# kcleal/fslr

Hardware: AMD Instinct MI355X
Metric: Jaccard pair-compares/sec + HBM GB/s vs roofline, 1M-read interval cluster (higher is better)
Workload: dtype int32

## Files before the change

### fslr_amd/csrc/capi.hip

```cpp
#include <algorithm>
#include <atomic>
#include <cstdint>
#include <cstdlib>
#include <cstring>
#include <string>
#include <thread>
#include <vector>

#include "fslr_hip.h"
#include "ctx.hpp"
#include "kernels.hpp"

using namespace fslr;

namespace {

int alloc_errw(fslr_ctx* c, int cap);

int ensure_capacity(fslr_ctx* c, int64_t n, int64_t ni, int n_chroms) {
  int rc;
  if (n > c->cap_n) {
    if ((rc = dalloc(c, &c->rmeta, n)) || (rc = dalloc(c, &c->rlen8, n)) || (rc = dalloc(c, &c->fwd, n)) ||
        (rc = dalloc(c, &c->parent, n)) || (rc = dalloc(c, &c->forest, n)) ||
        (rc = dalloc(c, &c->heavy, n)) ||
// ... 740 lines not shown
  b.rmeta = c->rmeta;
  b.iv = c->iv;
  b.shard = c->shard;
  b.n_shards = c->n_shards;
  b.dchrom = c->filter_active ? c->fdchrom : c->have_data_pos ? c->dchrom : nullptr;
  b.drec = c->filter_active ? c->fdrec : c->have_data_pos ? c->drec : nullptr;
  b.dgate = c->filter_active ? c->fdgate : c->dgate;
  b.data_pos = c->data_pos;
  b.chist = c->chist;
  b.keys = c->keys;
  b.keys2 = c->keys2;
  b.vals = c->vals;
  b.vals2 = c->vals2;
  b.s_start = c->s_start;
  b.endkey = c->endkey;
  b.pmaxkey = c->pmaxkey;
  b.temp = c->temp;
  b.temp_bytes = c->temp_bytes;
  b.crange = c->filter_active ? c->crange_f : c->crange;
  b.qpos = c->qpos;
  b.rng_s = c->rng_s;
  b.swin = c->swin;
  b.tile_tests = nullptr;
  b.idx4 = c->idx4;
  b.idx_gate = c->idx_gate;
  return b;
}

__global__ void k_peek(const unsigned long long* counters, const int* err, long long* out) {
  if (threadIdx.x == 0) {
    out[0] = static_cast<long long>(counters[kEdgeCount]);
    out[1] = err[0];
    out[2] = err[3];
    out[3] = err[kErrZdCount];
  }
}

int fslr::peek_counts(fslr_ctx* c, long long out[4]) {
  if (!c->sw_total) {
    HIP_TRY(c, hipHostMalloc(reinterpret_cast<void**>(&c->sw_total), 16 * sizeof(long long), hipHostMallocMapped));
    HIP_TRY(c, hipHostGetDevicePointer(reinterpret_cast<void**>(&c->sw_total_dev), c->sw_total, 0));
  }
  k_peek<<<1, 64, 0, c->stream>>>(c->counters, c->errw, c->sw_total_dev + 4);
  HIP_TRY(c, hipGetLastError());
  HIP_TRY(c, hipStreamSynchronize(c->stream));
  const volatile long long* v = c->sw_total + 4;
// ... 34 lines not shown
int fslr::ensure_walk_index(fslr_ctx* c) {
  if (!c->index_built || c->index_full) return FSLR_OK;
  if (c->filter_active) return fail(c, FSLR_ERR_STATE, "the walk engine needs every chromosome's index");
  if (int rc = ensure_keys(c, false)) return rc;
  HIP_TRY(c, launch_index_walk_parts(index_bufs(c), static_cast<int>(c->n), static_cast<int>(c->ni), c->stream));
  c->index_full = true;
  return FSLR_OK;
}

extern "C" {

int fslr_build_index(fslr_ctx* c) {
  if (!c) return FSLR_ERR_INVALID;
  if (!c->reads_set) return fail(c, FSLR_ERR_STATE, "fslr_set_reads first");
  HIP_TRY(c, hipSetDevice(c->device));
  if (c->prof_phases) HIP_TRY(c, hipEventRecord(c->ev[0], c->stream));
  const bool full = !c->filter_active && !(c->have_data_pos && c->n_chroms <= 64 && c->n_shards == 1);
  const int nch = c->filter_active ? c->n_chroms_f : c->n_chroms;
  IndexBufs ib = index_bufs(c);
  const bool tt = !full && ib.dchrom && nch <= 64 && c->n_shards == 1;
  c->idx_tt_valid = false;
  if (tt) {
    const int64_t tiles = (c->ni_idx + 63) / 64 + 1;
    if (tiles > c->idx_tt_cap) {
      if (int rc = dalloc(c, &c->idx_tt, tiles)) return rc;
      c->idx_tt_cap = tiles;
    }
    ib.tile_tests = c->idx_tt;
  }
  HIP_TRY(c, launch_build_index(ib, static_cast<int>(c->n), static_cast<int>(c->ni_idx), nch, full, c->stream));
  c->idx_tt_valid = tt;
  c->index_lean = !full && index_bufs(c).dchrom && nch <= 64;
  c->lean_keys = false;
  c->lean_starts = false;
  c->built_n_chroms = nch;
  if (c->prof_phases) HIP_TRY(c, hipEventRecord(c->ev[1], c->stream));
  c->t_index_rec = c->prof_phases;
  c->index_built = true;
  ++c->index_gen;
  c->index_full = full;
  c->bwd_ranges = full;
  c->built_shard = c->shard;
  c->built_n_shards = c->n_shards;
  return FSLR_OK;
}

static int query_impl(fslr_ctx* c, const fslr_params* p, int64_t a_begin, int64_t a_end, int shard, int n_shards);

int fslr_query(fslr_ctx* c, const fslr_params* p, int64_t a_begin, int64_t a_end) {
  if (!c || !p || !p->pass_table) return FSLR_ERR_INVALID;
  if (a_begin < 0 || a_end > c->n || a_begin > a_end) return fail(c, FSLR_ERR_INVALID, "bad read range");
// ... 46 lines not shown
  if ((rc = ensure_grp(c))) return rc;
  s.grp = c->grp;
  s.rmeta = c->rmeta;
  s.rlen8 = c->rlen8;
  s.idx4 = c->idx4;
  s.idx_gate = c->idx_gate;
  s.rng_s = c->rng_s;
  s.swin = c->swin;
  s.umax = c->umax;
  s.ni = static_cast<int>(nix);
  if (c->filter_active && c->pf_on && c->pf_thr_gen != c->thr_gen)
    return fail(c, FSLR_ERR_STATE, "the thresholds changed after fslr_set_position_filter: plan the range again");
  s.nq = c->filter_active && c->pf_on ? static_cast<int>(c->pf_hi - c->pf_lo) : static_cast<int>(nix);
  s.n_reads = static_cast<int>(c->n);
  s.a_begin = static_cast<int>(a_begin);
  s.a_end = static_cast<int>(a_end);
  s.qlen_cut = p->qlen_cut;
  s.nal_cut = p->nal_cut;
  s.lb = c->lbounds;
  s.tile_cnt = c->sw_tile;
  s.tile_off = c->sw_tile + c->sw_tiles;
  s.tests_ready = c->idx_tt_valid && s.nq == static_cast<int>(nix);
  s.tile_tests = s.tests_ready ? c->idx_tt : c->sw_tile + 2 * c->sw_tiles;
  s.tile_ub = c->sw_tile + 3 * c->sw_tiles;
  s.edges = c->edges;
  s.edge_iu = c->edge_iu;
  s.edge_cap = c->edge_cap;
  s.fwd = c->fwd;
  s.counters = c->counters;
  s.err = c->errw;
  s.wstat = c->sw_wstat;
  s.wstat_waves = c->sw_wstat_waves;
  s.wlo = c->sw_wlo;
  s.n_ent = 0;
  s.n_dev = nullptr;
  s.ent_cap = c->ent_cap;
  for (int k = 0; k < 5; ++k) s.ev[k] = c->prof_phases ? c->sw_ev[k] : nullptr;
  s.ev[0] = nullptr;
  s.hist_mat = nullptr;
  s.hist_mod = 0;
  if (coarse) sweep_coarse_hist(s);
  if (dest_n > 0) sweep_dest_hist(s, dest_n, dest_shift);
  s.dest_totals = dest_n > 0 ? c->part_cnt : nullptr;
  if (!c->reuse || c->lb_gen != c->input_gen || c->lb_q != p->qlen_cut || c->lb_n != p->nal_cut) {
    HIP_TRY(c, launch_len_bounds(c->rmeta, 0, static_cast<int>(c->n), p->qlen_cut, p->nal_cut, c->lbounds, c->stream));
    c->lb_gen = c->input_gen;
    c->lb_q = p->qlen_cut;
    c->lb_n = p->nal_cut;
  }
  mode = count_only ? 0 : 2;
  for (int attempt = 0; attempt < 3; ++attempt) {
    s.ent = c->ent;
    s.ent_sorted = c->ent_sorted;
    s.ent_ub = c->ent_ub;
    s.ub_cap = c->ent_ub_cap;
    s.temp = c->sweep_temp;
    s.temp_bytes = c->sweep_temp_bytes;
    if (mode == 2) HIP_TRY(c, launch_sweep_plan(s, c->stream));
    s.k0 = e0;
    s.k1 = e1;
    s.p0 = s.p1 = nullptr;
    if (c->prof_phases) HIP_TRY(c, hipEventRecord(c->sw_ev[0], c->stream));
    const bool fast = c->reuse && !defer && mode == 2 && attempt == 0 && c->sw_prev_gen == c->input_gen &&
                      c->sw_prev_a0 == a_begin && c->sw_prev_a1 == a_end && c->sw_prev_q == p->qlen_cut &&
                      c->sw_prev_nc == p->nal_cut && c->sw_prev_umax == c->umax_host && c->sw_prev_n > 0 &&
                      c->sw_prev_n <= c->ent_cap && c->sw_prev_n < (int64_t(1) << 31) && !c->filter_active;
    long long* n_dev = reinterpret_cast<long long*>(c->counters + kSwNdev);
// ... 42 lines not shown
  s.temp = c->sweep_temp;
  s.temp_bytes = c->sweep_temp_bytes;
  return FSLR_OK;
}

static int sweep_impl(fslr_ctx* c, const fslr_params* p, int64_t a_begin, int64_t a_end, hipEvent_t e0,
                      hipEvent_t e1) {
  SweepArgs s{};
  int mode = 2;
  int rc = sweep_front(c, p, a_begin, a_end, e0, e1, s, mode, false, true);
  if (rc) return rc;
  if (e0) {
    const int slot = static_cast<int>(c->n_kern2++ % fslr_ctx::kKernRing);
    s.p0 = c->kev2[2 * slot];
    s.p1 = c->kev2[2 * slot + 1];
  }
  s.parent = c->parent;
  HIP_TRY(c, launch_sweep_pairs(s, mode, c->stream));
  c->hooked = true;
  c->sw_ev_rec = c->prof_phases;
  return FSLR_OK;
}

static int prepare_query(fslr_ctx* c, const fslr_params* p, bool keep_sticky = false) {
  HIP_TRY(c, hipSetDevice(c->device));
  if (c->edge_cap == 0) {
    int rc = fslr_reserve_edges(c, std::max<int64_t>(1 << 16, 12 * c->n));
    if (rc) return rc;
  }
  if (c->defer_cap == 0) {
    int rc = fslr_reserve_deferred(c, std::max<int64_t>(1 << 20, c->n));
    if (rc) return rc;
  }
  c->umax_host.assign(FSLR_MAX_L, 0);
  for (int I = 1; I <= FSLR_MAX_L; ++I) {
    const unsigned char* row = p->pass_table + (I - 1) * kPassStride;
    int um = 0;
    for (int U = I; U <= kPassStride; ++U)
      if (row[U - 1]) um = U;
    for (int U = I; U <= um; ++U)
      if (!row[U - 1]) return fail(c, FSLR_ERR_INVALID, "pass_table row is not a prefix in U");
    c->umax_host[I - 1] = um;
  }
  if (c->umax_host != c->umax_dev_copy) {
    c->umax_dev_copy = c->umax_host;
    HIP_TRY(c, hipMemcpyAsync(c->umax, c->umax_dev_copy.data(), FSLR_MAX_L * sizeof(int), hipMemcpyHostToDevice,
                              c->stream));
  }
  if (!c->wstat) {
    const int w = query_max_waves();
    int rc = dalloc(c, &c->wstat, static_cast<size_t>(w) * kWStride);
    if (rc) return rc;
    c->wstat_waves = w;
  }
  HIP_TRY(c, launch_query_reset(c->counters, kNumCounters, c->errw, keep_sticky ? kErrKeep : kErrWords, c->fwd,
                                c->parent, static_cast<int>(c->n), c->stream));
  c->hooked = false;
  std::memset(&c->cap_stats, 0, sizeof(c->cap_stats));
  if (!keep_sticky) c->zd_lost = false;
  c->edges_global = false;
  c->cap_gmode = false;
  c->last_qcut = p->qlen_cut;
  c->last_ncut = p->nal_cut;
  c->q_thr = p->edge_threshold;
  c->zd_host = true;
  return FSLR_OK;
}

static int query_impl(fslr_ctx* c, const fslr_params* p, int64_t a_begin, int64_t a_end, int shard, int n_shards) {
  if (!c->index_built) return fail(c, FSLR_ERR_STATE, "fslr_build_index first");
  if (c->filter_active)
    return fail(c, FSLR_ERR_STATE, "the index covers a chromosome subset (fslr_set_chrom_filter): use "
                                   "fslr_sweep_partition / fslr_sweep_evaluate");
  if (int rc = prepare_query(c, p)) return rc;
  c->zd_host = n_shards > 1;
  QueryArgs g;
  g.rmeta = c->rmeta;
  g.iv = c->iv;
  g.qpos = c->qpos;
  g.rng_s = c->rng_s;
  g.idx4 = c->idx4;
  g.idx_gate = c->idx_gate;
  g.defer = c->defer;
  g.defer_cap = c->defer_cap;
  g.umax = c->umax;
  g.lb = c->lbounds;
  c->lb_gen = -1;
  g.qlen_cut = p->qlen_cut;
  g.nal_cut = p->nal_cut;
  g.a_begin = static_cast<int>(a_begin);
  g.a_end = static_cast<int>(a_end);
  g.shard = shard;
  g.n_shards = n_shards;
  g.edges = c->edges;
  g.edge_iu = c->edge_iu;
  g.edge_cap = c->edge_cap;
  g.fwd = c->fwd;
  g.heavy = c->heavy;
  g.counters = c->counters;
  g.err = c->errw;
  g.mode = c->ablate & 3;
  g.diag = c->diag;
  g.wstat = c->wstat;
  g.wstat_waves = c->wstat_waves;
  g.ev_k0 = g.ev_k1 = nullptr;
  if (c->profiling && c->n > 0 && a_end > a_begin) {
    const int slot = static_cast<int>(c->n_kern++ % fslr_ctx::kKernRing);
    g.ev_k0 = c->kev[2 * slot];
    g.ev_k1 = c->kev[2 * slot + 1];
  }
  c->last_full = a_begin == 0 && a_end == c->n && n_shards == 1;
  c->last_qcut = p->qlen_cut;
  c->last_ncut = p->nal_cut;
  const int want = p->flags & 3;
  const bool sweep_ok = c->thr_mode == 0 && !c->any_zero_aln && n_shards == 1;
  if (want == FSLR_ENGINE_SWEEP && !sweep_ok)
    return fail(c, FSLR_ERR_INVALID, "the sweep engine needs overlap thresholds >= 1, no aln_size == 0 interval "
                                     "and one query shard");
  const bool sweep = want == FSLR_ENGINE_SWEEP || (want == FSLR_ENGINE_AUTO && sweep_ok && c->last_full);
  c->last_engine = sweep ? FSLR_ENGINE_SWEEP : FSLR_ENGINE_WALK;
  if (c->prof_phases) HIP_TRY(c, hipEventRecord(c->ev[2], c->stream));
  if (!sweep) {
    int rc = ensure_walk_index(c);
    if (rc) return rc;
  }
  if (sweep) {
    int rc = sweep_impl(c, p, a_begin, a_end, g.ev_k0, g.ev_k1);
    if (rc) return rc;
  } else {
    HIP_TRY(c, launch_query(g, c->thr_mode, c->stream));
  }
  if (c->prof_phases) HIP_TRY(c, hipEventRecord(c->ev[3], c->stream));
  c->t_query_rec = c->prof_phases;
  c->t_kernel_rec = c->profiling && c->n > 0 && a_end > a_begin;
  return FSLR_OK;
}

int fslr_set_chrom_filter(fslr_ctx* c, const uint8_t* owned) {
  if (c) c->pf_on = false;
  if (c) ++c->input_gen;
  if (!c) return FSLR_ERR_INVALID;
  if (!c->reads_set) return fail(c, FSLR_ERR_STATE, "fslr_set_reads first");
// ... 630 lines not shown
```

### fslr_amd/csrc/ctx.hpp

```cpp
#pragma once
#include <cstdint>
#include <string>
#include <vector>

#include "fslr_hip.h"
#include "kernels.hpp"

struct fslr_ctx {
  int device = 0;
  hipStream_t stream = nullptr;
  bool own_stream = false;
  std::string err;
  int64_t n = 0, ni = 0;
  int n_chroms = 0;
  int thr_mode = 0;
  bool reads_set = false, index_built = false, have_data_pos = false;
  bool hooked = false;
  bool index_full = false;
  bool bwd_ranges = false;
  bool index_lean = false;
  bool lean_keys = false;
  bool lean_starts = false;
  int built_n_chroms = 0;
  bool filter_active = false;
// ... 40 lines not shown
  int4* idx4 = nullptr;
  int2* idx_gate = nullptr;
  unsigned long long* defer = nullptr;
  int64_t defer_cap = 0;
  int* data_pos = nullptr;
  unsigned* dchrom = nullptr;
  int4* drec = nullptr;
  int2* dgate = nullptr;
  int* chist = nullptr;
  int* s_start = nullptr;
  int2* crange = nullptr;
  unsigned long long* keys = nullptr;
  unsigned long long* keys2 = nullptr;
  int* vals = nullptr;
  int* vals2 = nullptr;
  unsigned long long* endkey = nullptr;
  unsigned long long* pmaxkey = nullptr;
  void* temp = nullptr;
  size_t temp_bytes = 0;
  int* umax = nullptr;
  int4* lbounds = nullptr;
  int64_t lb_gen = -1;
  double lb_q = 0.0, lb_n = 0.0;
  int2* edges = nullptr;
  unsigned short* edge_iu = nullptr;
  int64_t edge_cap = 0;
  int* fwd = nullptr;
  int* heavy = nullptr;
  int* parent = nullptr;
  int* upl = nullptr;
  int64_t upl_cap = 0;
  unsigned long long* upl64 = nullptr;
  int64_t upl64_cap = 0;
  int2* forest = nullptr;
  unsigned long long* forest_cnt = nullptr;
  int* forest_blk = nullptr;
  unsigned long long* counters = nullptr;
  unsigned long long* wstat = nullptr;
  int wstat_waves = 0;
  unsigned long long* diag = nullptr;
  int* errw = nullptr;
  long long* rows_col = nullptr;
  int64_t rows_cap = 0, rows_n = 0, rows_codes = 0, rows_cids = 0;
  long long* rows_ord = nullptr;
  unsigned char* rows_keep = nullptr;
  int* rows_int = nullptr;
// ... 6 lines not shown
  std::vector<int64_t> rows_cid;
  int zd_cap = 0;
  bool zd_lost = false;
  bool zd_host = false;
  int q_thr = 0;
  long long* sw_tile = nullptr;
  long long* sw_total = nullptr;
  long long* sw_total_dev = nullptr;
  unsigned long long* ent_ub = nullptr;
  int64_t ent_ub_cap = 0;
  int64_t sw_tiles = 0;
  unsigned long long* sw_wstat = nullptr;
  int* sw_wlo = nullptr;
  int sw_wstat_waves = 0;
  hipEvent_t sw_ev[5] = {};
  bool sw_ev_rec = false;
  unsigned long long* ent = nullptr;
  unsigned long long* ent_sorted = nullptr;
  int64_t ent_cap = 0;
  void* sweep_temp = nullptr;
  size_t sweep_temp_bytes = 0;
  bool any_zero_aln = false;
  long long* idx_tt = nullptr;
  int64_t idx_tt_cap = 0;
  bool idx_tt_valid = false;
  bool reuse = true;
  uint64_t input_gen = 1;
  uint64_t sw_prev_gen = 0;
  double sw_prev_q = 0, sw_prev_nc = 0;
  std::vector<int> sw_prev_umax;
  int64_t sw_prev_a0 = -1, sw_prev_a1 = -1, sw_prev_n = 0;
  bool sw_fast_used = false;
  int last_engine = FSLR_ENGINE_WALK;
  int* thr_tmp = nullptr;
  int64_t cap_n = 0, cap_ni = 0, cap_chroms = 0;
  std::vector<int> umax_host, umax_dev_copy;
  std::vector<unsigned char> aln_zero_host;
  int ablate = 0;
  bool last_full = false;
  double last_qcut = 0.0, last_ncut = 0.0;
  fslr_cap_stats cap_stats = {};
  bool edges_global = false;
  bool cap_gmode = false;
  struct CapWork* capw = nullptr;
  struct SearchWork* srw = nullptr;
  uint64_t index_gen = 0;
// ... 79 lines not shown
```

### fslr_amd/csrc/index.hip

```cpp
#include <hipcub/hipcub.hpp>

#include "kernels.hpp"
#include "wave.hpp"

namespace fslr {
namespace {

constexpr int kRangeBlock = 256;
constexpr int kRangeSpan = 1024;
constexpr int kTile = 256;
constexpr int kWin = 512;
constexpr int kLeanHalo = kWin;

__global__ void k_keys_csr(const int4* __restrict__ rmeta, const int4* __restrict__ iv, int n,
                           unsigned long long* __restrict__ keys64, int* __restrict__ vals) {
  for (int r = blockIdx.x * blockDim.x + threadIdx.x; r < n; r += gridDim.x * blockDim.x) {
    const int4 m = rmeta[r];
    const int len = m.y & 0xffff;
    for (int j = 0; j < len; ++j) {
      const int k = m.x + j;
      const int4 rec = iv[k];
      keys64[k] = (static_cast<unsigned long long>(rec.x) << 32) | static_cast<unsigned>(rec.y);
      vals[k] = (r << 6) | j;
    }
// ... 280 lines not shown
  }
  m = threadIdx.x > 0 ? part[threadIdx.x - 1] : 0ull;
  for (int i = b; i < e; ++i) {
    const unsigned long long tot = group[i];
    group[i] = m;
    m = max_u64(m, tot);
  }
}

struct TilePrefix {
  const unsigned long long* loc;
  const unsigned long long* group_excl;
  __device__ __forceinline__ unsigned long long incl(int t) const { return max_u64(group_excl[t / kGroup], loc[t]); }
};

template <bool kBwd>
__global__ __launch_bounds__(kRangeBlock) void k_ranges(const int4* __restrict__ idx4, int shard, int n_shards,
                                                        const int* __restrict__ s_start,
                                                        const unsigned long long* __restrict__ endkey,
                                                        TilePrefix tile_incl,
                                                        const int2* __restrict__ crange, int ni,
                                                        int2* __restrict__ rng_s, int* __restrict__ swin,
                                                        const int2* __restrict__ gate, int n_chroms = 0,
                                                        long long* __restrict__ tile_tests = nullptr) {
  __shared__ int w_st[kBwd ? kRangeSpan + 2 * kWin : kRangeSpan + kLeanHalo];
  __shared__ int w_pm[kBwd ? kRangeSpan + kWin : 1];
  __shared__ unsigned long long t_part[kBwd ? kRangeBlock : 1];
  __shared__ int c_beg[kBwd ? 1 : 64];
  const int q0 = blockIdx.x * kRangeSpan;
  if constexpr (!kBwd)
    if (threadIdx.x < 64) c_beg[threadIdx.x] = threadIdx.x < n_chroms ? crange[threadIdx.x].x : 0x7FFFFFFF;
  const int w0 = kBwd ? max(q0 - kWin, 0) : q0;
  const int w1 = min(q0 + kRangeSpan + (kBwd ? kWin : kLeanHalo), ni);
  const int wp1 = min(q0 + kRangeSpan, ni);
  constexpr int kPerQ = kRangeSpan / kRangeBlock;
  int4 pre4[kPerQ];
  int2 preg[kPerQ];
  if constexpr (kBwd) {
    for (int t = threadIdx.x; t < w1 - w0; t += kRangeBlock) w_st[t] = s_start[w0 + t];
  } else {
#pragma unroll
    for (int u = 0; u < kPerQ; ++u) {
      const int q = q0 + threadIdx.x + u * kRangeBlock;
      pre4[u] = q < wp1 ? idx4[q] : make_int4(0, 0, 0, 0);
      preg[u] = q < wp1 ? gate[q] : make_int2(0, 0);
    }
    for (int t = kRangeSpan + threadIdx.x; t < w1 - w0; t += kRangeBlock) w_st[t] = idx4[w0 + t].x;
#pragma unroll
    for (int u = 0; u < kPerQ; ++u) w_st[threadIdx.x + u * kRangeBlock] = pre4[u].x;
  }
  if constexpr (kBwd) {
// ... 2 lines not shown
    unsigned long long m = 0ull;
    for (int u = 0; u < kPer; ++u) {
      const int p = w0 + threadIdx.x * kPer + u;
      k[u] = p < wp1 ? endkey[p] : 0ull;
      m = max_u64(m, k[u]);
    }
    t_part[threadIdx.x] = m;
    __syncthreads();
    for (int o = 1; o < kRangeBlock; o <<= 1) {
      const unsigned long long v = threadIdx.x >= o ? t_part[threadIdx.x - o] : 0ull;
      __syncthreads();
      t_part[threadIdx.x] = max_u64(t_part[threadIdx.x], v);
      __syncthreads();
    }
    m = w0 > 0 ? tile_incl.incl(w0 / kTile - 1) : 0ull;
    if (threadIdx.x > 0) m = max_u64(m, t_part[threadIdx.x - 1]);
    for (int u = 0; u < kPer; ++u) {
      m = max_u64(m, k[u]);
      w_pm[threadIdx.x * kPer + u] = static_cast<int>(static_cast<unsigned>(m));
    }
  }
  __syncthreads();
  if constexpr (!kBwd) {
#pragma unroll
    for (int u = 0; u < kPerQ; ++u) {
      const int q = q0 + threadIdx.x + u * kRangeBlock;
      const int4 rq = pre4[u];
      int m = 0;
      if (q < wp1 && (n_shards == 1 || shard_owns(rq.w >> 6, shard, n_shards))) {
        const int e = rq.y;
        int c = 0;
#pragma unroll
        for (int b = 32; b > 0; b >>= 1)
          if (c + b < 64 && c_beg[c + b] <= q) c += b;
        const int2 cr = crange[c];
        const int2 gq = preg[u];
        const int key = gq.x != 0 && (gq.y & 0xFFFFFF) != 0 ? min(e, e - rq.z) : e;
        const int hi_lim = min(cr.y, w1);
        int lo = q + 1, hi = hi_lim;
        while (lo < hi) {
          const int mid = (lo + hi) >> 1;
          if (w_st[mid - w0] <= key) lo = mid + 1; else hi = mid;
        }
        if (lo == hi_lim && hi_lim < cr.y) {
          int step = 1;
          hi = lo;
          while (hi < cr.y && idx4[hi].x <= key) {
            lo = hi + 1;
            hi = lo + step;
            step <<= 1;
          }
          if (hi > cr.y) hi = cr.y;
          while (lo < hi) {
            const int mid = (lo + hi) >> 1;
            if (idx4[mid].x <= key) lo = mid + 1; else hi = mid;
          }
        }
        m = lo - q - 1;
        swin[q] = m;
      }
      if (tile_tests) {
        const int tot = rdl(wave_incl_scan(m), kWave - 1);
        const int tq = q0 + (threadIdx.x & ~(kWave - 1)) + u * kRangeBlock;
        if ((threadIdx.x & (kWave - 1)) == 0 && tq < wp1) tile_tests[tq / kWave] = tot;
      }
    }
    return;
  }
#pragma unroll
  for (int u = 0; u < kPerQ; ++u) {
    const int q = q0 + threadIdx.x + u * kRangeBlock;
    if (q >= wp1) break;
    const int4 rq = kBwd ? make_int4(0, 0, 0, 0) : pre4[u];
    if (n_shards > 1 && !shard_owns((kBwd ? idx4[q].w : rq.w) >> 6, shard, n_shards)) continue;
    int c, e;
    if constexpr (kBwd) {
      const unsigned long long ek = endkey[q];
      c = static_cast<int>(ek >> 32);
      e = static_cast<int>(static_cast<unsigned>(ek));
    } else {
      e = rq.y;
      c = 0;
#pragma unroll
      for (int b = 32; b > 0; b >>= 1)
        if (c + b < 64 && c_beg[c + b] <= q) c += b;
    }
    const int2 cr = crange[c];
// ... 125 lines not shown
  k_tile_max<<<grid_for(ni, kTile), kTile, 0, s>>>(b.endkey, ni, b.pmaxkey);
  return launch_walk_parts(b, 0, ni, s, false);
}

hipError_t launch_index_walk_parts(const IndexBufs& b, int n, int ni, hipStream_t s) {
  if (ni <= 0) return hipSuccess;
  return launch_walk_parts(b, n, ni, s, true);
}

hipError_t launch_build_index(const IndexBufs& b, int n, int ni, int n_chroms, bool full, hipStream_t s) {
  if (ni <= 0) return hipSuccess;
  hipError_t e;
  size_t tb = b.temp_bytes;
  if (b.dchrom && n_chroms <= kMaxFusedChroms) {
    const int rounds = chrom_rounds(ni);
    const int ntl = static_cast<int>((static_cast<long long>(ni) + rounds * kTileThreads - 1) / (rounds * kTileThreads));
    k_chrom_count<<<ntl, kTileThreads, 0, s>>>(b.dchrom, ni, ntl, rounds, b.chist);
    k_chrom_scan<<<n_chroms, 1024, 0, s>>>(b.chist, ntl, b.crange);
    if (!full) {
      k_chrom_scatter<false><<<ntl, kTileThreads, 0, s>>>(b.dchrom, b.drec, b.dgate, b.chist, ni, ntl, rounds, b.idx4,
                                                          b.idx_gate, nullptr, b.endkey, b.vals);
      k_ranges<false><<<(ni + kRangeSpan - 1) / kRangeSpan, kRangeBlock, 0, s>>>(
          b.idx4, b.shard, b.n_shards, nullptr, nullptr,
          TilePrefix{nullptr, nullptr}, b.crange, ni, b.rng_s, b.swin, b.idx_gate, n_chroms, b.tile_tests);
      return hipGetLastError();
    }
    k_chrom_scatter<true><<<ntl, kTileThreads, 0, s>>>(b.dchrom, b.drec, b.dgate, b.chist, ni, ntl, rounds, b.idx4, b.idx_gate,
                                                       b.s_start, b.endkey, b.vals);
    return launch_walk_parts(b, n, ni, s, true);
  } else if (b.dchrom) {
    unsigned* k32 = reinterpret_cast<unsigned*>(b.keys2);
    e = hipcub::DeviceRadixSort::SortPairs(b.temp, tb, b.dchrom, k32, b.drec, b.idx4, ni, 0, bits_for(n_chroms), s);
    if (e != hipSuccess) return e;
    k_finish<false><<<grid_for(ni, kTile), kTile, 0, s>>>(b.idx4, k32, b.rmeta, ni, b.idx_gate, b.s_start, b.endkey,
                                                          b.pmaxkey, b.qpos, b.shard, b.n_shards);
  } else {
    k_keys_csr<<<grid_for(n), 256, 0, s>>>(b.rmeta, b.iv, n, b.keys, b.vals);
    e = hipcub::DeviceRadixSort::SortPairs(b.temp, tb, b.keys, b.keys2, b.vals, b.vals2, ni, 0,
                                           32 + bits_for(n_chroms), s);
    if (e != hipSuccess) return e;
    k_gather_records<<<grid_for(ni), 256, 0, s>>>(b.vals2, b.iv, b.rmeta, ni, b.idx4);
    k_finish<true><<<grid_for(ni, kTile), kTile, 0, s>>>(b.idx4, b.keys2, b.rmeta, ni, b.idx_gate, b.s_start, b.endkey,
                                                         b.pmaxkey, b.qpos, b.shard, b.n_shards);
  }
  return launch_walk_parts(b, n, ni, s, false);
}

// ... 79 lines not shown
```

### fslr_amd/csrc/kernels.hpp

```cpp
#pragma once
#include <hip/hip_runtime.h>

#include <cassert>
#include <cstddef>
#include <cstdint>

#ifdef FSLR_DEBUG_BOUNDS
#define FSLR_BOUND(i, n) assert(static_cast<long long>(i) >= 0 && static_cast<long long>(i) < static_cast<long long>(n))
#else
#define FSLR_BOUND(i, n) ((void)0)
#endif

namespace fslr {

constexpr int kWave = 64;
constexpr int kPassStride = 128;
constexpr int kMaxCoord = 1 << 30;
constexpr int kShardShift = 6;
constexpr int kErrWords = 8;
constexpr int kErrOverflow = 4;
constexpr int kErrZdCount = 6;
constexpr int kErrSticky = 7;
constexpr int kErrKeep = 6;
constexpr int kErrZdCap = 8;
// ... 16 lines not shown
               kSwTests = kQueueBase2 + 8 * kQueueStride,
               kSwNdev = kSwTests + 8,
               kNumCounters = kSwTests + 16 };
enum WaveStat { kWsEval = 0, kWsJacc, kWsCand, kWsAlgoBytes, kWsOverflow, kWsMatchEntries, kWsMatchedPairs,
                kWsMaxFwd, kWsWalked, kWsBase = 9, kWsProf = kWsBase + 16, kWStride = 32 };

__device__ __forceinline__ bool thr_ok(int o, int t) { return t >= 0 ? o >= t : o <= ~t; }

__device__ __forceinline__ bool iv_match_general(int sa, int ea, int ta, int sb, int eb, int tb) {
  const int o = max(min(ea, eb) - max(sa, sb), 0);
  return thr_ok(o, ta) && thr_ok(o, tb);
}

__device__ __forceinline__ bool lengths_pass(int q1, int q2, int n1, int n2, double qcut, double ncut, bool* zd) {
  int mn = min(q1, q2), mx = max(q1, q2);
  if (mx == 0) { *zd = true; return false; }
  if (static_cast<double>(mn) / static_cast<double>(mx) >= qcut) return true;
  mn = min(n1, n2);
  mx = max(n1, n2);
  if (mx == 0) { *zd = true; return false; }
  return static_cast<double>(mn) / static_cast<double>(mx) >= ncut;
}

struct IndexBufs {
  int shard, n_shards;
  const int4* rmeta;
  const int4* iv;
  const unsigned* dchrom;
  const int4* drec;
  const int2* dgate;
  const int* data_pos;
  int* chist;
  unsigned long long* keys;
  unsigned long long* keys2;
  int* vals;
  int* vals2;
  int* s_start;
  unsigned long long* endkey;
  unsigned long long* pmaxkey;
  void* temp;
  size_t temp_bytes;
  const int2* crange;
  int* qpos;
  int2* rng_s;
  int* swin;
  long long* tile_tests;
  int4* idx4;
  int2* idx_gate;
};
hipError_t index_temp_bytes(int ni, size_t* bytes, hipStream_t s);
hipError_t launch_build_index(const IndexBufs& b, int n_reads, int ni, int n_chroms, bool full, hipStream_t s);
hipError_t launch_index_rescatter(const IndexBufs& b, int ni, int n_chroms, hipStream_t s);
hipError_t launch_index_swin(const IndexBufs& b, int ni, hipStream_t s);
hipError_t launch_index_endkeys(const IndexBufs& b, int ni, int n_chroms, hipStream_t s);
hipError_t launch_index_walk_parts(const IndexBufs& b, int n_reads, int ni, hipStream_t s);
hipError_t launch_index_bwd_ranges(const IndexBufs& b, int ni, hipStream_t s);
hipError_t launch_set_thr(const int* thr, int4* iv, const int* qpos, int4* idx4, const int* data_pos,
                          int4* drec, int ni, hipStream_t s);

struct QueryArgs {
  const int4* rmeta;
  const int4* iv;
  const int* qpos;
  const int2* rng_s;
  const int4* idx4;
  const int2* idx_gate;
  const int* umax;
  int4* lb;
  double qlen_cut, nal_cut;
  int a_begin, a_end;
  int shard, n_shards;
  int nv;
  int k_static;
  int pass_records;
  int* heavy;
  int2* edges;
  unsigned short* edge_iu;
  long long edge_cap;
  int* fwd;
  unsigned long long* defer;
  long long defer_cap;
  unsigned long long* counters;
  int* err;
  int mode;
  unsigned long long* wstat;
  int wstat_waves;
  unsigned long long* diag;
  hipEvent_t ev_k0, ev_k1;
};
hipError_t launch_query(const QueryArgs& a, int thr_mode, hipStream_t s);
hipError_t launch_len_bounds(const int4* rmeta, int a0, int a1, double qcut, double ncut, int4* lb, hipStream_t s);
int query_max_waves();

struct SweepArgs {
  const int4* rmeta;
  const unsigned char* rlen8;
  const int4* idx4;
  const int2* idx_gate;
  const int2* rng_s;
  const int* swin;
  const int* umax;
  int ni, n_reads;
  int nq;
  int a_begin, a_end;
  double qlen_cut, nal_cut;
  int4* lb;
  long long* tile_cnt;
  long long* tile_off;
  long long* tile_tests;
  bool tests_ready;
  long long* tile_ub;
  unsigned long long* ent_ub;
  long long ub_cap;
  unsigned long long* ent;
  unsigned long long* ent_sorted;
  unsigned long long* ent_mid;
  unsigned long long* pair_scr;
  int* grp;
  int* hist_mat;
  int hist_lo, hist_h;
  int hist_mod;
  long long* dest_totals;
  long long n_ent;
  const long long* n_dev;
  long long ent_cap;
  void* temp;
  size_t temp_bytes;
  int2* edges;
  unsigned short* edge_iu;
  long long edge_cap;
  int* fwd;
  int* parent;
  unsigned long long* counters;
// ... 106 lines not shown
```

### fslr_amd/csrc/query.hip

```cpp
#include "fslr_hip.h"
#include <algorithm>
#include <cstdlib>
#include <type_traits>

#include "kernels.hpp"
#include "wave.hpp"

namespace fslr {
namespace {

constexpr int kWavesPerBlock = 4;
constexpr int kShardMask = (1 << kShardShift) - 1;
constexpr int kBlock = kWave * kWavesPerBlock;
constexpr int kStageCap = kWave;
constexpr int kChunk = 8;
constexpr int kDynamicMinReads = 64;
constexpr int kHashBits = 9;
constexpr int kHashSize = 1 << kHashBits;
constexpr int kHashLimit = 320;
constexpr int kMatchCap = 192;
constexpr int kPassRecords = 512;
constexpr unsigned kEpochShift = 25;
constexpr unsigned kEpochMax = 127;
constexpr unsigned kBMask = 0x1FFFFFFu;
// ... 4 lines not shown
constexpr unsigned kStConflict = 16u;
constexpr unsigned kDefPair = 0u;
constexpr unsigned kDefWitness = 1u;

#ifdef FSLR_SECTION_PROF
#define SEC_NOW(v) const unsigned long long v = __builtin_amdgcn_s_memtime()
#define SEC_ADD(k, t0) (sec[k] += __builtin_amdgcn_s_memtime() - (t0))
constexpr int kSections = 8;
#else
#define SEC_NOW(v) (void)0
#define SEC_ADD(k, t0) (void)0
#endif

__device__ __forceinline__ int part_of(int B, int npass) {
  return static_cast<int>(((static_cast<unsigned>(B) * 0x85EBCA6Bu) >> 8) % static_cast<unsigned>(npass));
}

__global__ void k_len_bounds(const int4* __restrict__ rmeta, int a0, int a1, double qcut, double ncut,
                             int4* __restrict__ lb) {
  for (int a = a0 + blockIdx.x * blockDim.x + threadIdx.x; a < a1; a += gridDim.x * blockDim.x) {
    const int4 m = rmeta[a];
    const int2 q = ratio_range(m.z, qcut), n = ratio_range(m.w, ncut);
    lb[a] = make_int4(q.x, q.y, n.x, n.y);
  }
}

struct DeferStage {
  unsigned long long* DQ;
  int n;
  __device__ void flush(const QueryArgs& g, int nb, int lane) {
    wave_lds_sync();
    const bool act = lane < nb;
    const unsigned long long e = act ? DQ[lane] : 0ull;
    const int rem = n - nb;
    const unsigned long long mv = lane < rem ? DQ[nb + lane] : 0ull;
    wave_lds_sync();
    if (lane < rem) DQ[lane] = mv;
    n = rem;
    unsigned long long base = 0;
    if (lane == 0) base = atomicAdd(&g.counters[kDeferCount], static_cast<unsigned long long>(nb));
    base = __shfl(base, 0);
    const long long k = static_cast<long long>(base) + lane;
    if (act && k < g.defer_cap) g.defer[k] = e;
  }
  __device__ void put(const QueryArgs& g, bool p, int a, int B, int ic, int jc, unsigned kind, int lane) {
    const unsigned long long m = __ballot(p);
// ... 584 lines not shown
  if (cached) return cached;
  int dev = 0, cus = 256, per_cu = 0;
  if (hipGetDevice(&dev) == hipSuccess) (void)hipDeviceGetAttribute(&cus, hipDeviceAttributeMultiprocessorCount, dev);
  if (hipOccupancyMaxActiveBlocksPerMultiprocessor(&per_cu, query_kernel<kThrMode, kMulti>, kBlock, 0) != hipSuccess ||
      per_cu < 1)
    per_cu = 4;
  cached = cus * per_cu;
  return cached;
}

}

int query_max_waves() {
  const int b = std::max(std::max(resident_blocks<0, false>(), resident_blocks<1, false>()),
                         std::max(resident_blocks<0, true>(), resident_blocks<1, true>()));
  return b * kWavesPerBlock;
}

hipError_t launch_len_bounds(const int4* rmeta, int a0, int a1, double qcut, double ncut, int4* lb, hipStream_t s) {
  if (a1 > a0) k_len_bounds<<<grid_for(a1 - a0), 256, 0, s>>>(rmeta, a0, a1, qcut, ncut, lb);
  return hipGetLastError();
}

hipError_t launch_query(const QueryArgs& a_in, int thr_mode, hipStream_t s) {
  QueryArgs a = a_in;
  const long long span = static_cast<long long>(a.a_end) - a.a_begin;
  {
    const long long nb = (span + kShardMask) >> kShardShift;
    const long long m = nb > a.shard ? (nb - 1 - a.shard) / a.n_shards + 1 : 0;
    long long nv = m << kShardShift;
    if (m > 0 && a.shard + (m - 1) * a.n_shards == nb - 1 && (span & kShardMask)) nv -= kWave - (span & kShardMask);
    a.nv = static_cast<int>(nv);
  }
  const long long nq = a.nv;
  if (span > 0) {
    k_len_bounds<<<grid_for(span), 256, 0, s>>>(a.rmeta, a.a_begin, a.a_end, a.qlen_cut, a.nal_cut, a.lb);
    const long long nchunks = (nq + kChunk - 1) / kChunk;
    long long want = (nchunks + kWavesPerBlock - 1) / kWavesPerBlock;
#ifdef FSLR_SECTION_PROF
    if (const char* e = getenv("FSLR_QUERY_BLOCKS")) want = std::min(want, std::max(1ll, atoll(e)));
#endif
    const int cap = thr_mode == 0 ? resident_blocks<0, false>() : resident_blocks<1, false>();
    const int blocks = static_cast<int>(want < cap ? want : cap);
    if (blocks * kWavesPerBlock > a.wstat_waves) return hipErrorInvalidValue;
    if (blocks > 0) {
      const long long nw = static_cast<long long>(blocks) * kWavesPerBlock;
// ... 32 lines not shown
```

### fslr_amd/csrc/sweep.hip

```cpp
#include <hipcub/hipcub.hpp>
#include <cstdio>
#include <cstdlib>
#include <cstring>
#include <type_traits>

#include "fslr_hip.h"
#include "kernels.hpp"
#include "wave.hpp"

namespace fslr {
namespace {

constexpr int kSwWaves = 4;
constexpr int kSwBlock = kSwWaves * kWave;
constexpr int kPairLimit = 64;
constexpr int kPerPass = 40;
constexpr int kWsFields = 4;

__device__ __forceinline__ int entry_a(unsigned long long e) { return static_cast<int>(e >> 39); }
__device__ __forceinline__ unsigned long long above(int h) { return h >= 63 ? 0ull : (~0ull << (h + 1)); }
__device__ __forceinline__ unsigned long long upto(int h) { return h >= 63 ? ~0ull : ((2ull << h) - 1); }

__device__ __forceinline__ int part_of(int B, int npass) {
  return static_cast<int>(((static_cast<unsigned>(B) * 0x85EBCA6Bu) >> 8) % static_cast<unsigned>(npass));
// ... 374 lines not shown
    if (static_cast<int>(threadIdx.x) < H) {
      const long long k0 = static_cast<long long>(threadIdx.x) * P, k1 = k0 + P - 1;
      dtot[threadIdx.x] = static_cast<long long>(off[k1]) + mat[k1] - off[k0];
    }
  }
}

__global__ __launch_bounds__(256) void k_wave_bounds(const long long* __restrict__ ub, const long long* __restrict__ tests,
                                                     int nt, int nw, int* __restrict__ wlo) {
  const long long total = ub[nt - 1] + tests[nt - 1] + static_cast<long long>(nt) * kTileCost;
  auto wave_of = [&](int t) -> int {
    const long long c = ub[t] + static_cast<long long>(t) * kTileCost;
    return total > 0 ? static_cast<int>(min(static_cast<long long>(nw - 1), c * nw / total)) : 0;
  };
  for (int t = blockIdx.x * blockDim.x + threadIdx.x; t < nt; t += gridDim.x * blockDim.x) {
    const int w = t == 0 ? 0 : wave_of(t);
    const int wp = t == 0 ? -1 : wave_of(t - 1);
    for (int x = wp + 1; x <= w; ++x) wlo[x] = t;
    if (t == nt - 1)
      for (int x = w + 1; x <= nw; ++x) wlo[x] = nt;
  }
}

__global__ __launch_bounds__(256) void k_tile_tests(const int* __restrict__ swin, int ni, long long* __restrict__ tests) {
  const int nt = (ni + kWave - 1) / kWave;
  const int lane = lane_id();
  for (int t = (blockIdx.x * blockDim.x + threadIdx.x) >> 6; t < nt; t += (gridDim.x * blockDim.x) >> 6) {
    const int q = t * kWave + lane;
    int v = q < ni ? swin[q] : 0;
    v = wave_incl_scan(v);
    if (lane == kWave - 1) tests[t] = v;
  }
}

__global__ __launch_bounds__(256) void k_compact(const unsigned long long* __restrict__ src,
                                                 const long long* __restrict__ ub, const long long* __restrict__ off,
                                                 const long long* __restrict__ cnt, int nt,
                                                 unsigned long long* __restrict__ dst) {
  const int lane = lane_id();
  for (int t = (blockIdx.x * blockDim.x + threadIdx.x) >> 6; t < nt; t += (gridDim.x * blockDim.x) >> 6) {
    const long long n = cnt[t], a = ub[t], b = off[t];
    for (long long k = lane; k < n; k += kWave) dst[b + k] = src[a + k];
  }
}

constexpr int kChunk2 = 512;
// ... 950 lines not shown

}

int sweep_max_waves() {
  return std::max(std::max(blocks_mode(0), blocks_mode(1)), std::max(blocks_mode(2), blocks_pairs())) * kSwWaves;
}

size_t sweep_temp_bytes(long long ent_cap, long long ni, hipStream_t s) {
  size_t a = 0, b = 0, c = 0;
  (void)hipcub::DeviceScan::ExclusiveSum(nullptr, c, static_cast<int*>(nullptr), static_cast<int*>(nullptr),
                                         kGrpInts / 2, s);
  (void)hipcub::DeviceRadixSort::SortKeys(nullptr, a, static_cast<unsigned long long*>(nullptr),
                                          static_cast<unsigned long long*>(nullptr), static_cast<int>(ent_cap), 39,
                                          64, s);
  (void)hipcub::DeviceScan::ExclusiveSum(nullptr, b, static_cast<long long*>(nullptr),
                                         static_cast<long long*>(nullptr), static_cast<int>((ni + kWave - 1) / kWave),
                                         s);
  return std::max(std::max(a, b), c);
}

hipError_t launch_sweep_plan(const SweepArgs& a, hipStream_t s) {
  const int nt = tiles_of(a);
  if (nt == 0) return hipSuccess;
  if (!a.tests_ready)
    k_tile_tests<<<grid_for(static_cast<long long>(nt) * kWave, 256, 4096), 256, 0, s>>>(a.swin, a.nq, a.tile_tests);
  size_t tb = a.temp_bytes;
  hipError_t e = hipcub::DeviceScan::ExclusiveSum(a.temp, tb, a.tile_tests, a.tile_ub, nt, s);
  if (e != hipSuccess) return e;
  const int nw = sweep_blocks(nt) * kSwWaves;
  if (!a.wlo || nw > a.wstat_waves) return hipErrorInvalidValue;
  k_wave_bounds<<<grid_for(nt, 256, 1024), 256, 0, s>>>(a.tile_ub, a.tile_tests, nt, nw, a.wlo);
  return hipGetLastError();
}

hipError_t launch_sweep_count(const SweepArgs& a0, int mode, long long* total_dev, hipStream_t s, long long* n_dev,
                              long long cap) {
  const SweepArgs& a = a0;
  const int nt = tiles_of(a);
  if (nt == 0) return hipMemsetAsync(total_dev, 0, 3 * sizeof(long long), s);
  const int blocks = mode == 2 ? sweep_blocks(nt) : std::min(blocks_mode(mode), (nt + kSwWaves - 1) / kSwWaves);
  if (blocks * kSwWaves > a.wstat_waves) return hipErrorInvalidValue;
  if (a.k0) (void)hipEventRecord(a.k0, s);
  if (mode == 2)
    k_sweep<2><<<blocks, kSwBlock, 0, s>>>(a);
  else
    k_sweep<0><<<blocks, kSwBlock, 0, s>>>(a);
  if (a.k1) (void)hipEventRecord(a.k1, s);
  if (mode == 2) {
    const bool fuse = dest_scan_fused(a, blocks);
    k_sweep_total<<<1, 1024, 0, s>>>(a.wstat, blocks * kSwWaves, a.tile_ub, a.tile_tests, nt, a.counters, a.err,
                                     total_dev, n_dev, cap, fuse ? a.hist_mat : nullptr, a.grp + kGrpInts / 2,
                                     a.hist_h, blocks, a.dest_totals);
    if (a.ev[1]) (void)hipEventRecord(a.ev[1], s);
// ... 192 lines not shown
```

Before: 39.20 billion.

## Fuse sweep planning scan with wave bounds and merge length bounds into query reset

The index build now also emits per-block sums of tile test counts. The sweep planner can then run one kernel that forms the exclusive scan and the wave boundaries, replacing the hipcub scan plus a separate wave-bounds kernel. Separately, the query reset kernel is fused with the length-bounds computation when the sweep engine will run, and a freshness flag skips the later len_bounds launch. This cuts kernel launches and passes over memory in the query prologue, at the cost of each plan block redundantly re-reading all block sums and more state tracking.

Result: slower. 38.71 billion (-1.3%).

```diff
diff --git a/fslr_amd/csrc/capi.hip b/fslr_amd/csrc/capi.hip
--- a/fslr_amd/csrc/capi.hip
+++ b/fslr_amd/csrc/capi.hip
@@ -786,6 +786,7 @@
   b.rng_s = c->rng_s;
   b.swin = c->swin;
   b.tile_tests = nullptr;
+  b.blk_tests = nullptr;
   b.idx4 = c->idx4;
   b.idx_gate = c->idx_gate;
   return b;
@@ -866,11 +867,13 @@
   c->idx_tt_valid = false;
   if (tt) {
     const int64_t tiles = (c->ni_idx + 63) / 64 + 1;
-    if (tiles > c->idx_tt_cap) {
-      if (int rc = dalloc(c, &c->idx_tt, tiles)) return rc;
-      c->idx_tt_cap = tiles;
+    const int64_t groups = (tiles + kPlanBlkTiles - 1) / kPlanBlkTiles + 1;
+    if (tiles + groups > c->idx_tt_cap) {
+      if (int rc = dalloc(c, &c->idx_tt, tiles + groups)) return rc;
+      c->idx_tt_cap = tiles + groups;
     }
     ib.tile_tests = c->idx_tt;
+    ib.blk_tests = c->idx_bt = c->idx_tt + tiles;
   }
   HIP_TRY(c, launch_build_index(ib, static_cast<int>(c->n), static_cast<int>(c->ni_idx), nch, full, c->stream));
   c->idx_tt_valid = tt;
@@ -963,6 +966,7 @@
   s.tile_off = c->sw_tile + c->sw_tiles;
   s.tests_ready = c->idx_tt_valid && s.nq == static_cast<int>(nix);
   s.tile_tests = s.tests_ready ? c->idx_tt : c->sw_tile + 2 * c->sw_tiles;
+  s.blk_tests = s.tests_ready ? c->idx_bt : nullptr;
   s.tile_ub = c->sw_tile + 3 * c->sw_tiles;
   s.edges = c->edges;
   s.edge_iu = c->edge_iu;
@@ -983,7 +987,9 @@
   if (coarse) sweep_coarse_hist(s);
   if (dest_n > 0) sweep_dest_hist(s, dest_n, dest_shift);
   s.dest_totals = dest_n > 0 ? c->part_cnt : nullptr;
-  if (!c->reuse || c->lb_gen != c->input_gen || c->lb_q != p->qlen_cut || c->lb_n != p->nal_cut) {
+  if (c->lb_fresh && c->lb_gen == c->input_gen && c->lb_q == p->qlen_cut && c->lb_n == p->nal_cut) {
+    c->lb_fresh = false;
+  } else if (!c->reuse || c->lb_gen != c->input_gen || c->lb_q != p->qlen_cut || c->lb_n != p->nal_cut) {
     HIP_TRY(c, launch_len_bounds(c->rmeta, 0, static_cast<int>(c->n), p->qlen_cut, p->nal_cut, c->lbounds, c->stream));
     c->lb_gen = c->input_gen;
     c->lb_q = p->qlen_cut;
@@ -1072,7 +1078,7 @@
   return FSLR_OK;
 }
 
-static int prepare_query(fslr_ctx* c, const fslr_params* p, bool keep_sticky = false) {
+static int prepare_query(fslr_ctx* c, const fslr_params* p, bool keep_sticky = false, bool with_bounds = false) {
   HIP_TRY(c, hipSetDevice(c->device));
   if (c->edge_cap == 0) {
     int rc = fslr_reserve_edges(c, std::max<int64_t>(1 << 16, 12 * c->n));
@@ -1103,8 +1109,20 @@
     if (rc) return rc;
     c->wstat_waves = w;
   }
-  HIP_TRY(c, launch_query_reset(c->counters, kNumCounters, c->errw, keep_sticky ? kErrKeep : kErrWords, c->fwd,
-                                c->parent, static_cast<int>(c->n), c->stream));
+  c->lb_fresh = false;
+  if (with_bounds && c->n > 0 &&
+      (!c->reuse || c->lb_gen != c->input_gen || c->lb_q != p->qlen_cut || c->lb_n != p->nal_cut)) {
+    HIP_TRY(c, launch_query_prologue(c->counters, kNumCounters, c->errw, keep_sticky ? kErrKeep : kErrWords, c->fwd,
+                                     c->parent, static_cast<int>(c->n), c->rmeta, p->qlen_cut, p->nal_cut,
+                                     c->lbounds, c->stream));
+    c->lb_gen = c->input_gen;
+    c->lb_q = p->qlen_cut;
+    c->lb_n = p->nal_cut;
+    c->lb_fresh = true;
+  } else {
+    HIP_TRY(c, launch_query_reset(c->counters, kNumCounters, c->errw, keep_sticky ? kErrKeep : kErrWords, c->fwd,
+                                  c->parent, static_cast<int>(c->n), c->stream));
+  }
   c->hooked = false;
   std::memset(&c->cap_stats, 0, sizeof(c->cap_stats));
   if (!keep_sticky) c->zd_lost = false;
@@ -1122,7 +1140,12 @@
   if (c->filter_active)
     return fail(c, FSLR_ERR_STATE, "the index covers a chromosome subset (fslr_set_chrom_filter): use "
                                    "fslr_sweep_partition / fslr_sweep_evaluate");
-  if (int rc = prepare_query(c, p)) return rc;
+  const int want = p->flags & 3;
+  const bool sweep_ok = c->thr_mode == 0 && !c->any_zero_aln && n_shards == 1;
+  const bool full_q = a_begin == 0 && a_end == c->n && n_shards == 1;
+  const bool sweep = want == FSLR_ENGINE_SWEEP || (want == FSLR_ENGINE_AUTO && sweep_ok && full_q);
+  c->lb_gen = -1;
+  if (int rc = prepare_query(c, p, false, sweep && sweep_ok)) return rc;
   c->zd_host = n_shards > 1;
   QueryArgs g;
   g.rmeta = c->rmeta;
@@ -1135,7 +1158,6 @@
   g.defer_cap = c->defer_cap;
   g.umax = c->umax;
   g.lb = c->lbounds;
-  c->lb_gen = -1;
   g.qlen_cut = p->qlen_cut;
   g.nal_cut = p->nal_cut;
   g.a_begin = static_cast<int>(a_begin);
@@ -1159,15 +1181,12 @@
     g.ev_k0 = c->kev[2 * slot];
     g.ev_k1 = c->kev[2 * slot + 1];
   }
-  c->last_full = a_begin == 0 && a_end == c->n && n_shards == 1;
+  c->last_full = full_q;
   c->last_qcut = p->qlen_cut;
   c->last_ncut = p->nal_cut;
-  const int want = p->flags & 3;
-  const bool sweep_ok = c->thr_mode == 0 && !c->any_zero_aln && n_shards == 1;
   if (want == FSLR_ENGINE_SWEEP && !sweep_ok)
     return fail(c, FSLR_ERR_INVALID, "the sweep engine needs overlap thresholds >= 1, no aln_size == 0 interval "
                                      "and one query shard");
-  const bool sweep = want == FSLR_ENGINE_SWEEP || (want == FSLR_ENGINE_AUTO && sweep_ok && c->last_full);
   c->last_engine = sweep ? FSLR_ENGINE_SWEEP : FSLR_ENGINE_WALK;
   if (c->prof_phases) HIP_TRY(c, hipEventRecord(c->ev[2], c->stream));
   if (!sweep) {
diff --git a/fslr_amd/csrc/ctx.hpp b/fslr_amd/csrc/ctx.hpp
--- a/fslr_amd/csrc/ctx.hpp
+++ b/fslr_amd/csrc/ctx.hpp
@@ -86,6 +86,7 @@
   int4* lbounds = nullptr;
   int64_t lb_gen = -1;
   double lb_q = 0.0, lb_n = 0.0;
+  bool lb_fresh = false;
   int2* edges = nullptr;
   unsigned short* edge_iu = nullptr;
   int64_t edge_cap = 0;
@@ -138,6 +139,7 @@
   size_t sweep_temp_bytes = 0;
   bool any_zero_aln = false;
   long long* idx_tt = nullptr;
+  long long* idx_bt = nullptr;
   int64_t idx_tt_cap = 0;
   bool idx_tt_valid = false;
   bool reuse = true;
diff --git a/fslr_amd/csrc/index.hip b/fslr_amd/csrc/index.hip
--- a/fslr_amd/csrc/index.hip
+++ b/fslr_amd/csrc/index.hip
@@ -326,11 +326,14 @@
                                                         const int2* __restrict__ crange, int ni,
                                                         int2* __restrict__ rng_s, int* __restrict__ swin,
                                                         const int2* __restrict__ gate, int n_chroms = 0,
-                                                        long long* __restrict__ tile_tests = nullptr) {
+                                                        long long* __restrict__ tile_tests = nullptr,
+                                                        long long* __restrict__ blk_tests = nullptr) {
+  static_assert(kRangeSpan == kPlanBlkTiles * kWave, "a block's tiles are one block sum of the sweep plan");
   __shared__ int w_st[kBwd ? kRangeSpan + 2 * kWin : kRangeSpan + kLeanHalo];
   __shared__ int w_pm[kBwd ? kRangeSpan + kWin : 1];
   __shared__ unsigned long long t_part[kBwd ? kRangeBlock : 1];
   __shared__ int c_beg[kBwd ? 1 : 64];
+  __shared__ long long b_part[kBwd ? 1 : kRangeBlock / kWave];
   const int q0 = blockIdx.x * kRangeSpan;
   if constexpr (!kBwd)
     if (threadIdx.x < 64) c_beg[threadIdx.x] = threadIdx.x < n_chroms ? crange[threadIdx.x].x : 0x7FFFFFFF;
@@ -379,6 +382,7 @@
   }
   __syncthreads();
   if constexpr (!kBwd) {
+    long long bt = 0;
 #pragma unroll
     for (int u = 0; u < kPerQ; ++u) {
       const int q = q0 + threadIdx.x + u * kRangeBlock;
@@ -420,6 +424,16 @@
         const int tot = rdl(wave_incl_scan(m), kWave - 1);
         const int tq = q0 + (threadIdx.x & ~(kWave - 1)) + u * kRangeBlock;
         if ((threadIdx.x & (kWave - 1)) == 0 && tq < wp1) tile_tests[tq / kWave] = tot;
+        bt += tot;
+      }
+    }
+    if (blk_tests) {
+      if ((threadIdx.x & (kWave - 1)) == 0) b_part[threadIdx.x / kWave] = bt;
+      __syncthreads();
+      if (threadIdx.x == 0) {
+        long long t = 0;
+        for (int k = 0; k < kRangeBlock / kWave; ++k) t += b_part[k];
+        blk_tests[blockIdx.x] = t;
       }
     }
     return;
@@ -591,7 +605,8 @@
                                                           b.idx_gate, nullptr, b.endkey, b.vals);
       k_ranges<false><<<(ni + kRangeSpan - 1) / kRangeSpan, kRangeBlock, 0, s>>>(
           b.idx4, b.shard, b.n_shards, nullptr, nullptr,
-          TilePrefix{nullptr, nullptr}, b.crange, ni, b.rng_s, b.swin, b.idx_gate, n_chroms, b.tile_tests);
+          TilePrefix{nullptr, nullptr}, b.crange, ni, b.rng_s, b.swin, b.idx_gate, n_chroms, b.tile_tests,
+          b.tile_tests ? b.blk_tests : nullptr);
       return hipGetLastError();
     }
     k_chrom_scatter<true><<<ntl, kTileThreads, 0, s>>>(b.dchrom, b.drec, b.dgate, b.chist, ni, ntl, rounds, b.idx4, b.idx_gate,
diff --git a/fslr_amd/csrc/kernels.hpp b/fslr_amd/csrc/kernels.hpp
--- a/fslr_amd/csrc/kernels.hpp
+++ b/fslr_amd/csrc/kernels.hpp
@@ -62,6 +62,7 @@
   return static_cast<double>(mn) / static_cast<double>(mx) >= ncut;
 }
 
+constexpr int kPlanBlkTiles = 16;
 struct IndexBufs {
   int shard, n_shards;
   const int4* rmeta;
@@ -85,6 +86,7 @@
   int2* rng_s;
   int* swin;
   long long* tile_tests;
+  long long* blk_tests;
   int4* idx4;
   int2* idx_gate;
 };
@@ -130,6 +132,8 @@
 };
 hipError_t launch_query(const QueryArgs& a, int thr_mode, hipStream_t s);
 hipError_t launch_len_bounds(const int4* rmeta, int a0, int a1, double qcut, double ncut, int4* lb, hipStream_t s);
+hipError_t launch_query_prologue(unsigned long long* counters, int nc, int* err, int ne, int* fwd, int* parent, int n,
+                                 const int4* rmeta, double qcut, double ncut, int4* lb, hipStream_t s);
 int query_max_waves();
 
 struct SweepArgs {
@@ -149,6 +153,7 @@
   long long* tile_off;
   long long* tile_tests;
   bool tests_ready;
+  const long long* blk_tests;
   long long* tile_ub;
   unsigned long long* ent_ub;
   long long ub_cap;
diff --git a/fslr_amd/csrc/query.hip b/fslr_amd/csrc/query.hip
--- a/fslr_amd/csrc/query.hip
+++ b/fslr_amd/csrc/query.hip
@@ -50,6 +50,21 @@
     const int4 m = rmeta[a];
     const int2 q = ratio_range(m.z, qcut), n = ratio_range(m.w, ncut);
     lb[a] = make_int4(q.x, q.y, n.x, n.y);
+  }
+}
+
+__global__ void k_query_prologue(unsigned long long* __restrict__ counters, int nc, int* __restrict__ err, int ne,
+                                 int* __restrict__ fwd, int* __restrict__ parent, int n,
+                                 const int4* __restrict__ rmeta, double qcut, double ncut, int4* __restrict__ lb) {
+  const int i = blockIdx.x * blockDim.x + threadIdx.x;
+  if (i < nc) counters[i] = 0ull;
+  if (i < ne) err[i] = 0;
+  for (int k = i; k < n; k += gridDim.x * blockDim.x) {
+    const int4 m = rmeta[k];
+    fwd[k] = 0;
+    if (parent) parent[k] = k;
+    const int2 q = ratio_range(m.z, qcut), r = ratio_range(m.w, ncut);
+    lb[k] = make_int4(q.x, q.y, r.x, r.y);
   }
 }
 
@@ -680,6 +695,13 @@
   return hipGetLastError();
 }
 
+hipError_t launch_query_prologue(unsigned long long* counters, int nc, int* err, int ne, int* fwd, int* parent, int n,
+                                 const int4* rmeta, double qcut, double ncut, int4* lb, hipStream_t s) {
+  const long long work = std::max<long long>(std::max(nc, ne), n);
+  k_query_prologue<<<grid_for(work), 256, 0, s>>>(counters, nc, err, ne, fwd, parent, n, rmeta, qcut, ncut, lb);
+  return hipGetLastError();
+}
+
 hipError_t launch_query(const QueryArgs& a_in, int thr_mode, hipStream_t s) {
   QueryArgs a = a_in;
   const long long span = static_cast<long long>(a.a_end) - a.a_begin;
diff --git a/fslr_amd/csrc/sweep.hip b/fslr_amd/csrc/sweep.hip
--- a/fslr_amd/csrc/sweep.hip
+++ b/fslr_amd/csrc/sweep.hip
@@ -420,6 +420,56 @@
   }
 }
 
+constexpr int kPlanThreads = 1024;
+static_assert(kPlanThreads % kPlanBlkTiles == 0, "a plan block starts on a block sum");
+__global__ __launch_bounds__(kPlanThreads) void k_sweep_plan(const long long* __restrict__ tests,
+                                                             const long long* __restrict__ blk, int nt, int nblk,
+                                                             int nw, long long* __restrict__ ub,
+                                                             int* __restrict__ wlo) {
+  __shared__ long long red[3][kPlanThreads / kWave];
+  const int tid = threadIdx.x, lane = tid & (kWave - 1), w = tid >> 6;
+  const int t = blockIdx.x * kPlanThreads + tid;
+  const long long v = t < nt ? tests[t] : 0, vp = t > 0 && t < nt ? tests[t - 1] : 0;
+  const int b0 = blockIdx.x * (kPlanThreads / kPlanBlkTiles);
+  long long pre = 0, all = 0;
+  for (int k = tid; k < nblk; k += kPlanThreads) {
+    const long long x = blk[k];
+    all += x;
+    pre += k < b0 ? x : 0;
+  }
+  long long inc = v;
+  for (int o = 1; o < kWave; o <<= 1) {
+    const long long y = __shfl_up(inc, o);
+    if (lane >= o) inc += y;
+  }
+  for (int o = 32; o > 0; o >>= 1) {
+    pre += __shfl_xor(pre, o);
+    all += __shfl_xor(all, o);
+  }
+  if (lane == kWave - 1) red[0][w] = inc;
+  if (lane == 0) {
+    red[1][w] = pre;
+    red[2][w] = all;
+  }
+  __syncthreads();
+  long long base = 0, total = static_cast<long long>(nt) * kTileCost;
+  for (int x = 0; x < kPlanThreads / kWave; ++x) {
+    base += red[1][x] + (x < w ? red[0][x] : 0);
+    total += red[2][x];
+  }
+  if (t >= nt) return;
+  const long long u = base + inc - v;
+  ub[t] = u;
+  auto wave_of = [&](long long c) -> int {
+    return total > 0 ? static_cast<int>(min(static_cast<long long>(nw - 1), c * nw / total)) : 0;
+  };
+  const int wt = t == 0 ? 0 : wave_of(u + static_cast<long long>(t) * kTileCost);
+  const int wp = t == 0 ? -1 : wave_of(u - vp + static_cast<long long>(t - 1) * kTileCost);
+  for (int x = wp + 1; x <= wt; ++x) wlo[x] = t;
+  if (t == nt - 1)
+    for (int x = wt + 1; x <= nw; ++x) wlo[x] = nt;
+}
+
 __global__ __launch_bounds__(256) void k_tile_tests(const int* __restrict__ swin, int ni, long long* __restrict__ tests) {
   const int nt = (ni + kWave - 1) / kWave;
   const int lane = lane_id();
@@ -1416,13 +1466,18 @@
 hipError_t launch_sweep_plan(const SweepArgs& a, hipStream_t s) {
   const int nt = tiles_of(a);
   if (nt == 0) return hipSuccess;
+  const int nw = sweep_blocks(nt) * kSwWaves;
+  if (!a.wlo || nw > a.wstat_waves) return hipErrorInvalidValue;
+  if (a.tests_ready && a.blk_tests) {
+    k_sweep_plan<<<(nt + kPlanThreads - 1) / kPlanThreads, kPlanThreads, 0, s>>>(
+        a.tile_tests, a.blk_tests, nt, (nt + kPlanBlkTiles - 1) / kPlanBlkTiles, nw, a.tile_ub, a.wlo);
+    return hipGetLastError();
+  }
   if (!a.tests_ready)
     k_tile_tests<<<grid_for(static_cast<long long>(nt) * kWave, 256, 4096), 256, 0, s>>>(a.swin, a.nq, a.tile_tests);
   size_t tb = a.temp_bytes;
   hipError_t e = hipcub::DeviceScan::ExclusiveSum(a.temp, tb, a.tile_tests, a.tile_ub, nt, s);
   if (e != hipSuccess) return e;
-  const int nw = sweep_blocks(nt) * kSwWaves;
-  if (!a.wlo || nw > a.wstat_waves) return hipErrorInvalidValue;
   k_wave_bounds<<<grid_for(nt, 256, 1024), 256, 0, s>>>(a.tile_ub, a.tile_tests, nt, nw, a.wlo);
   return hipGetLastError();
 }
```
